# facebookresearch/jepa

Measured on AMD Instinct MI355X. Metric: V-JEPA pretrain clips/sec (fwd+bwd+EMA), higher is better.
Workload: dtype bf16; 1 GPU; V-JEPA pretrain step ViT-L/16 16x224x224, B=24/GPU, 2 multiblock masks (vitl16.yaml); global_batch=24, per_gpu_batch=24, parallelism=dp1, hw_queues=4

## Files before the change

include/vjepa_hip.h:

```cpp
#ifndef VJEPA_HIP_H
#define VJEPA_HIP_H

#include <stdint.h>

#ifdef __cplusplus
extern "C" {
#endif

typedef struct ihipStream_t* vj_stream_t;

int vj_abi_version(void);
const char* vj_last_error(void);

int vj_gather_rows(const void* src, void* dst, const int64_t* idx, int64_t B, int64_t K, int64_t row_bytes,
                   int64_t src_batch_stride_rows, vj_stream_t stream);
int vj_scatter_rows(const void* src, void* dst, const int64_t* idx, int64_t B, int64_t N, int64_t K,
                    int64_t row_bytes, vj_stream_t stream);
int vj_copy_rows(const void* src, void* dst, int64_t B, int64_t src_rows, int64_t src_off, int64_t dst_rows,
                 int64_t dst_off, int64_t n, int64_t D, vj_stream_t stream);

int vj_tubelet_pack(const float* clips, void* out_bf16, const int64_t* idx, int64_t B, int64_t C, int64_t T,
                    int64_t H, int64_t W, int64_t tubelet, int64_t patch, int64_t K, vj_stream_t stream);
int vj_add_pos(void* x_bf16, const float* pos, const int64_t* idx, int64_t B, int64_t K, int64_t D,
               vj_stream_t stream);
// ... 116 lines not shown

int vj_pred_assemble_fwd(const void* e_bf16, const float* mask_token, const float* pos, const int64_t* idx_e,
                         const int64_t* idx_p, void* out_bf16, int64_t B, int64_t Ke, int64_t Kp, int64_t D,
                         vj_stream_t stream);

int vj_target_rows(const void* x_bf16, const float* gamma, const float* beta, const int64_t* idx, float* h,
                   int64_t B, int64_t N, int64_t K, int64_t D, float eps_norm, float eps_ln, vj_stream_t stream);
int64_t vj_latent_loss_ws_bytes(void);
int vj_latent_loss(const void* z_bf16, const float* h, void* dz_bf16, int64_t numel, float p, float gscale,
                   float out_scale, int accumulate, float* loss_out, void* ws, int64_t ws_bytes,
                   vj_stream_t stream);
int vj_token_pstd(const void* z_bf16, float* pstd, float* stats ,
                  int64_t B, int64_t K, int64_t D, int accumulate, vj_stream_t stream);
int vj_reg_grad(const void* z_bf16, const float* pstd_sum, const float* stats, void* dz_bf16, int64_t B, int64_t K,
                int64_t D, int64_t n_masks, float coef, vj_stream_t stream);
int vj_reg_finish(const float* pstd_sum, int64_t n, int64_t n_masks, float* out, vj_stream_t stream);

int vj_adamw_ema(float* p, const float* g, float* exp_avg, float* exp_avg_sq, void* p_bf16, float* tgt,
                 void* tgt_bf16, int64_t n, float lr, float wd, float beta1, float beta2, float eps, int64_t step,
                 float gscale, float ema, vj_stream_t stream);
int vj_step_advance(const float* gstat, float* step_dev, vj_stream_t stream);
int vj_adamw_ema_guarded(float* p, const float* g, float* exp_avg, float* exp_avg_sq, void* p_bf16, float* tgt,
                         void* tgt_bf16, int64_t n, float lr, float wd, float beta1, float beta2, float eps, float gscale,
                         float ema, const float* gstat, int sel, float clip, float norm_scale, const float* step_dev,
                         vj_stream_t stream);
int64_t vj_grad_stats_chunks(void);
int vj_grad_stats_multi(const float* G, const float* M1, const float* M2, const int64_t* desc, int64_t n_tensors,
                        float* out, vj_stream_t stream);
int vj_ema_update(float* tgt, const float* src, void* tgt_bf16, int64_t n, float m, vj_stream_t stream);
int vj_cast_f32_to_bf16(const float* src, void* dst_bf16, int64_t n, vj_stream_t stream);
int64_t vj_sqnorm_ws_bytes(void);
int vj_sqnorm_f32(const float* g, int64_t n, float* out2, int accumulate, void* ws, int64_t ws_bytes,
                  vj_stream_t stream);

typedef struct vj_linear {
  const void* w;
  const float* b;
  const void* wT;
  int64_t ldwT;
  float* gw;
  float* gb;
  int64_t n_out, k_in;
} vj_linear_t;
typedef struct vj_norm {
  const float* g;
  const float* b;
  float* gg;
  float* gb;
} vj_norm_t;
typedef struct vj_block {
  vj_norm_t norm1;
  vj_linear_t qkv, proj;
  vj_norm_t norm2;
  vj_linear_t fc1, fc2;
} vj_block_t;
typedef void (*vj_layer_cb_t)(void* user, int layer);

int64_t vj_blocks_fwd_ws_bytes(int64_t M, int64_t D, int64_t Dh, int64_t heads, int64_t n_blocks, int save);
enum {
  VJ_GEMM_FLAGS_SEL_MASK = 0xffff,
  VJ_GEMM_FLAGS_FROM_SHIFT = 16,
  VJ_GEMM_FLAGS_FROM_MASK = 0xff
};
int vj_blocks_fwd(const vj_block_t* blocks, int64_t n_blocks, const void* x_in, void* x_out, int64_t M, int64_t D,
                  int64_t heads, const vj_seg_t* segs, int64_t n_segs, float ln_eps, int save, int gemm_flags, void* ws,
                  int64_t ws_bytes, vj_stream_t stream);
// ... 63 lines not shown
```

jepa_amd/csrc/optim.hip:

```cpp
#include "common.hpp"
#include "options.hpp"

struct AdamArgs {
  float* p;
  const float* g;
  float* m;
  float* v;
  bf16_t* p_bf16;
  float* tgt;
  bf16_t* tgt_bf16;
  int64_t n;
  float lr, wd, beta1, beta2, eps;
  float bc1, bc2_sqrt;
  float gscale;
  float ema;
  const float* gstat;
  int sel;
  float clip;
  float norm_scale;
  const float* step_dev;
};

template <bool SRC_ROUNDED>
__device__ __forceinline__ void ema4(float* tgt, bf16_t* tgt_bf16, int64_t q, float4 s, float m) {
// ... 144 lines not shown
    s += v.x * v.x + v.y * v.y + v.z * v.z + v.w * v.w;
    bad += (float)(!isfinite(v.x)) + (float)(!isfinite(v.y)) + (float)(!isfinite(v.z)) + (float)(!isfinite(v.w));
  }
  block4_stage(red, {s, bad});
  if (threadIdx.x == 0) {
    part[blockIdx.x] = block4_total(red[0]);
    part[SQ_BLOCKS + blockIdx.x] = block4_total(red[1]);
  }
}
__global__ __launch_bounds__(256) void sqnorm_finish_kernel(const float* __restrict__ part, float* __restrict__ out,
                                                            int accumulate) {
  __shared__ float red[2][4];
  float s = 0.f, bad = 0.f;
  for (int i = threadIdx.x; i < SQ_BLOCKS; i += 256) {
    s += part[i];
    bad += part[SQ_BLOCKS + i];
  }
  block4_stage(red, {s, bad});
  if (threadIdx.x == 0) {
    const float a = block4_total(red[0]), b = block4_total(red[1]);
    out[0] = accumulate ? out[0] + a : a;
    out[1] = accumulate ? out[1] + b : b;
  }
}
extern "C" int64_t vj_sqnorm_ws_bytes(void) { return 2 * SQ_BLOCKS * 4; }
extern "C" int vj_sqnorm_f32(const float* g, int64_t n, float* out2, int accumulate, void* ws, int64_t ws_bytes,
                             hipStream_t stream) {
  VJ_CHECK_ARG(n % 4 == 0, "vj_sqnorm_f32: n must be a multiple of 4");
  VJ_CHECK_ARG(ws_bytes >= vj_sqnorm_ws_bytes(), "vj_sqnorm_f32: workspace too small");
  hipLaunchKernelGGL(sqnorm_kernel, dim3(SQ_BLOCKS), dim3(256), 0, stream, g, n / 4, (float*)ws);
  VJ_LAUNCH_CHECK("vj_sqnorm_f32");
  hipLaunchKernelGGL(sqnorm_finish_kernel, dim3(1), dim3(256), 0, stream, (const float*)ws, out2, accumulate);
  VJ_LAUNCH_CHECK("vj_sqnorm_f32(finish)");
  return 0;
}

#define GS_CHUNKS 8
__global__ __launch_bounds__(256) void grad_stats_multi_kernel(const float* __restrict__ G, const float* __restrict__ M1,
                                                               const float* __restrict__ M2,
                                                               const int64_t* __restrict__ desc, float* __restrict__ out) {
  __shared__ float red[3][4];
  const int t = blockIdx.x, c = blockIdx.y;
  const int64_t off = desc[2 * t], n = desc[2 * t + 1];
  const int64_t per = cdiv64(cdiv64(n, GS_CHUNKS), 4) * 4;
  const int64_t lo = (int64_t)c * per, hi = lo + per < n ? lo + per : n;
  float s0 = 0.f, s1 = 0.f, s2 = 0.f;
  const int64_t n4 = hi > lo ? (hi - lo) >> 2 : 0;
  for (int64_t q = threadIdx.x; q < n4; q += 256) {
    const int64_t e = off + lo + 4 * q;
    const float4 g = *(const float4*)(G + e);
    s0 += g.x * g.x + g.y * g.y + g.z * g.z + g.w * g.w;
    if (M1) {
      const float4 a = *(const float4*)(M1 + e);
      const float4 b = *(const float4*)(M2 + e);
      s1 += fabsf(a.x) + fabsf(a.y) + fabsf(a.z) + fabsf(a.w);
      s2 += fabsf(b.x) + fabsf(b.y) + fabsf(b.z) + fabsf(b.w);
    }
  }
  for (int64_t e = lo + 4 * n4 + threadIdx.x; e < hi; e += 256) {
    const float g = G[off + e];
    s0 += g * g;
    if (M1) {
      s1 += fabsf(M1[off + e]);
      s2 += fabsf(M2[off + e]);
    }
  }
// ... 16 lines not shown
```

jepa_amd/engine/dp.py:

```python
import torch
import torch.distributed as dist

from .streams import independent_stream, side_stream


class GradReducer:
    def __init__(self, arena, vit, pred, world_size, overlap=True, pred_layers_per_bucket=4):
        self.arena = arena
        import os
        self.world = world_size
        self.enabled = world_size > 1 or (os.environ.get("VJ_FORCE_DP", "0") == "1" and dist.is_available()
                                          and dist.is_initialized())
        self.overlap = overlap
        self.coll_mode = os.environ.get("VJ_DP_COLL", "sync")
        if self.coll_mode not in ("sync", "async", "capi"):
            raise ValueError(f"VJ_DP_COLL={self.coll_mode!r}: expected sync, async or capi")
        self._capi = None
        self.extra_streams = []
        self.buckets = {}
        self.tail = []
        self._pending = []
        self.comm_stream = None
        self.launched = []
        self._exposed = []
        self.exposed_samples = 0
        if not self.enabled:
            return
        sl = arena.slots

        def span(prefix, names):
            offs = [sl[prefix + n] for n in names]
            return (min(s.off for s in offs), max(s.off + ((s.numel + 63) // 64) * 64 for s in offs))

        mats = ["attn.qkv.weight", "attn.proj.weight", "mlp.fc1.weight", "mlp.fc2.weight"]
        for li in range(len(vit.blocks)):
            self.buckets[("enc", li)] = [span(f"enc.blocks.{li}.", mats)]
        self.buckets[("enc", -1)] = [span("enc.", ["patch_embed.proj.weight"])]
        n_pred = len(pred.predictor_blocks)
        group = []
        for li in range(n_pred - 1, -1, -1):
            group.append(span(f"pred.predictor_blocks.{li}.", mats))
            if len(group) == pred_layers_per_bucket or li == 0:
                self.buckets[("pred", li)] = [(min(g[0] for g in group), max(g[1] for g in group))]
                group = []
        self.buckets[("pred", n_pred)] = [span("pred.", ["predictor_proj.weight"])]
        covered = sorted(r for rs in self.buckets.values() for r in rs)
        pos, total = 0, arena.total
        for lo, hi in covered:
            if lo > pos:
                self.tail.append((pos, lo))
            pos = max(pos, hi)
        if pos < total:
            self.tail.append((pos, total))
        self._diag = os.environ.get("VJ_DP_DIAG", "")
        self.coll_check = None
        if self.coll_mode == "capi" and not (arena.G.is_cuda and overlap):
            raise ValueError("VJ_DP_COLL=capi needs the gradient arena on a GPU and overlap_comm=True: the C-ABI collectives are "
                             "issued on the engine's communication stream")
        if (self.coll_mode == "capi" or self._diag == "extracomm") and arena.G.is_cuda:
            self._init_capi(arena.G.device)
            if self.coll_mode != "capi":
                self._capi_unused, self._capi = self._capi, None

    def _init_capi(self, device):
        import ctypes
        from ..hip.lib import check, load_library
        lib = load_library()
        n = lib.vj_comm_unique_id_bytes()
        idt = torch.zeros(n, dtype=torch.uint8, device=device)
        if dist.get_rank() == 0:
            buf = (ctypes.c_ubyte * n)()
            check(lib.vj_comm_unique_id(buf), "vj_comm_unique_id")
            idt.copy_(torch.tensor(list(buf), dtype=torch.uint8))
        dist.broadcast(idt, 0)
        raw = bytes(idt.cpu().tolist())
        handle = ctypes.c_void_p()
        check(lib.vj_comm_init(ctypes.byref(handle), dist.get_rank(), dist.get_world_size(), raw), "vj_comm_init")
        self._capi = (lib, handle)
        import weakref
        weakref.finalize(self, lib.vj_comm_destroy, handle)

    @property
    def route(self):
        if not (self.arena.G.is_cuda and self.overlap):
            return "blocking"
        return "capi" if self._capi is not None else self.coll_mode
# ... 79 lines not shown
            else:
                out["verdict"] = "comm-stream" if all(sid == marker for _, sid in colls) else "other-stream"
        except Exception as ex:
            out["error"] = f"{type(ex).__name__}: {ex}"[:200]
        return out

    def begin(self, producer_stream=None):
        if not self.enabled:
            return
        self.launched = []
        self._pending = []
        self._ev_next = 0
        self._producer = producer_stream
        if self.arena.G.is_cuda and self.overlap and self.comm_stream is None:
            self._pick_comm_stream()

    def _reduce(self, lo, hi, producer=None):
        g = self.arena.G[lo:hi]
        self.launched.append((lo, hi))
        if g.is_cuda and self.overlap:
            pool = self.__dict__.setdefault("_ev_pool", [])
            nxt = self.__dict__.get("_ev_next", 0)
            if nxt >= len(pool):
                pool.append(torch.cuda.Event())
            ev = pool[nxt]
            self._ev_next = nxt + 1
            ev.record(producer if producer is not None else torch.cuda.current_stream())
            self.comm_stream.wait_event(ev)
            if self._capi is not None:
                from ..hip.lib import check
                lib, handle = self._capi
                if self._diag != "skipcall":
                    check(lib.vj_comm_allreduce_bucket(handle, g.data_ptr(), g.numel(), self.comm_stream.cuda_stream), "vj_comm_allreduce_bucket")
                return
            with torch.cuda.stream(self.comm_stream):
                if self.coll_mode == "async":
                    self._pending.append(dist.all_reduce(g, op=dist.ReduceOp.SUM, async_op=True))
                else:
                    dist.all_reduce(g, op=dist.ReduceOp.SUM)
        else:
            dist.all_reduce(g, op=dist.ReduceOp.SUM)

    def layer_done(self, kind, layer):
        if not self.enabled:
            return
        for lo, hi in self.buckets.get((kind, layer), ()):
            self._reduce(lo, hi, getattr(self, "_producer", None))

    def finish(self):
        if not self.enabled:
            return
        for lo, hi in self.tail:
            self._reduce(lo, hi)
        if self.arena.G.is_cuda and self.overlap:
            cur = torch.cuda.current_stream()
            e0, e1 = torch.cuda.Event(enable_timing=True), torch.cuda.Event(enable_timing=True)
            e0.record(cur)
            for w in self._pending:
                w.wait()
            cur.wait_stream(self.comm_stream)
            e1.record(cur)
            self._exposed = (self._exposed + [(e0, e1)])[-16:]
        self._pending = []

    def exposed_ms(self):
        if not self._exposed:
            return None
        torch.cuda.synchronize()
        self.exposed_samples = len(self._exposed)
        return sum(a.elapsed_time(b) for a, b in self._exposed) / len(self._exposed)


# ... 7 lines not shown
```

jepa_amd/engine/step.py:

```python
import math
import os
import weakref

import torch

from ..hip import ops
from ..hip.lib import set_option
from . import chain, dp, optstate
from . import weights as _weights
from .layers import encoder_backward, encoder_forward, predictor_backward, predictor_forward
from .streams import device_index, independent_stream, low_priority_stream, side_stream
from .weights import FoldW, ParamArena, bump_generation, encoder_views, is_no_decay, predictor_views

_OVERLAP_FWD = os.environ.get("VJ_OVERLAP_FWD", "1") != "0"
_LN_FOLD = os.environ.get("VJ_LN_FOLD", "0") == "1"
_UPD_LOW_PRIO = os.environ.get("VJ_UPD_LOW_PRIO", "0") == "1"
_TGT_GEMM_FLAGS = int(os.environ.get("VJ_TGT_GEMM_FLAGS", "0"), 0)
_PRED_GEMM_FLAGS = int(os.environ.get("VJ_PRED_GEMM_FLAGS", "0"), 0)
_PRED_DGRAD_FLAGS = int(os.environ.get("VJ_PRED_DGRAD_FLAGS", "0"), 0)


class _TargetArena(ParamArena):

    def __init__(self, src: ParamArena, lo, hi, prefix, target_named_params, device):
        self.device = device
        self.slots = {n: s for n, s in src.slots.items() if n.startswith(prefix)}
        self.lo, self.hi = lo, hi
        self.P = torch.zeros(hi - lo, dtype=torch.float32, device=device)
        self.Pb = torch.zeros(hi - lo, dtype=torch.bfloat16, device=device)
        self.wT = {}
        self.frozen = {}
        for name, p in target_named_params:
            self.adopt(name, p)
        self.refresh_bf16()

    def make_folds(self, depth):
        self.folds = []
        for i in range(depth):
            wq, w1 = self.f32(f"enc.blocks.{i}.attn.qkv.weight"), self.f32(f"enc.blocks.{i}.mlp.fc1.weight")
            mk = lambda n: torch.empty(n, dtype=torch.float32, device=self.device)
            self.folds.append(FoldW(torch.empty_like(wq, dtype=torch.bfloat16), mk(wq.shape[0]), mk(wq.shape[0]),
                                    torch.empty_like(w1, dtype=torch.bfloat16), mk(w1.shape[0]), mk(w1.shape[0])))
        self.refresh_folds(0, depth)
        return self.folds

    def refresh_folds(self, b0, b1):
        if getattr(self, "folds", None) is None:
            return
        for i in range(b0, b1):
# ... 95 lines not shown
            if a not in self.arena.slots:
                p.data = p.data.to(device=dev, dtype=torch.float32).contiguous()
                self.tarena.frozen[a] = p.data
        self.tvit._hip_attach(self.tarena, "enc.")
        self.ew = encoder_views(self.arena, "enc.", self.vit,
                                self.arena.frozen["enc.pos_embed"].reshape(self.vit.num_patches, -1), train=True)
        self.pw = predictor_views(self.arena, "pred.", self.pred,
                                  self.arena.frozen["pred.predictor_pos_embed"].reshape(self.pred.num_patches, -1),
                                  train=True)
        self.tw = encoder_views(self.tarena, "enc.", self.tvit,
                                self.tarena.frozen["enc.pos_embed"].reshape(self.tvit.num_patches, -1), train=False)
        self._target_folds = None
        self.ln_fold_target = False
        if _LN_FOLD:
            self.set_ln_fold(True)
        def grp(named, nodecay):
            return [p for _, n, p in named if is_no_decay(n, p) == nodecay]
        self.param_groups = [
            {"params": grp(enc_named, False), "lr": 0.0, "weight_decay": 0.0, "_range": 0},
            {"params": grp(pred_named, False), "lr": 0.0, "weight_decay": 0.0, "_range": 2},
            {"params": grp(enc_named, True), "lr": 0.0, "weight_decay": 0, "WD_exclude": True, "_range": 1},
            {"params": grp(pred_named, True), "lr": 0.0, "weight_decay": 0, "WD_exclude": True, "_range": 3},
        ]
        self._slot_of = {id(sl.param): sl for sl in self.arena.slots.values()}
        self._step_dev = torch.zeros(1, dtype=torch.float32, device=dev)
        self._stat = torch.zeros(8, dtype=torch.float32, device=dev)
        self.reducer = dp.GradReducer(self.arena, self.vit, self.pred, world_size, overlap=overlap_comm)
        self.overlap_update = bool(overlap_update)
        self._upd_stream = self._make_update_stream() if self.overlap_update else None
        self.reducer.extra_streams = [self._upd_stream]
        self.reducer.prepare()
        self._gates = None
        self._plan = self._update_plan()

    @torch.no_grad()
    def forward_target(self, clips, masks_pred):
        B = clips.shape[0]
        self.tw.folds = self._target_folds if (self.ln_fold_target and self._target_folds is not None) else None
        x, _, _ = encoder_forward(self.tw, clips, None, save=False, final_norm=False, ws_tag=self._ws + "tgt",
                                  gemm_flags=_TGT_GEMM_FLAGS, gates=self._gate("enc"))
        N = self.tvit.num_patches
        return [ops.target_rows(x, self.tw.norm.g, self.tw.norm.b, mp, B, N, 1e-6, 1e-5) for mp in masks_pred]

    @torch.no_grad()
    def train_step(self, clips, masks_enc, masks_pred, lr, wd, ema, clip_now=False):
        assert len(masks_enc) == len(masks_pred), 'Currently require num encoder masks = num predictor masks'
        B = clips.shape[0]
        D = self.vit.embed_dim
        n_masks = len(masks_pred)
        mark = self._phase_mark
        mark('start')
        self._arena_stats = None
        mb = B if not self.micro_batch else min(int(self.micro_batch), B)
        chunks = [(c0, min(c0 + mb, B)) for c0 in range(0, B, mb)]
        numels = [B * mp.shape[1] * D for mp in masks_pred]
        nmin = min(numels)
        alpha = 1.0 / (nmin * n_masks)
        with_reg = self.reg_coeff != 0.0
        pstd = torch.empty((B, D), dtype=torch.float32, device=self.device)
        side = side_stream(self.device)
        hook = self.reducer.layer_done if self.reducer.enabled else None
        for ci, (c0, c1) in enumerate(chunks):
            last = ci == len(chunks) - 1
            beta = 0.0 if ci == 0 else 1.0
            cl = clips[c0:c1]
            me = [m[c0:c1] for m in masks_enc] if len(chunks) > 1 else masks_enc
            mp = [m[c0:c1] for m in masks_pred] if len(chunks) > 1 else masks_pred
            me = [m if m.is_contiguous() else m.contiguous() for m in me]
            mp = [m if m.is_contiguous() else m.contiguous() for m in mp]
            Bc = c1 - c0
            fwd_overlap = side.enabled and _OVERLAP_FWD
            if fwd_overlap:
                side.fork(cl, *mp)
                with torch.cuda.stream(side.stream):
                    h = self.forward_target(cl, mp)
            else:
                h = self.forward_target(cl, mp)
            z, segs, saved_e = encoder_forward(self.ew, cl, me, save=True, ws_tag=self._ws + "enc_save", gates=self._gate("enc"))
            zhat, tsegs, saved_p = predictor_forward(self.pw, z, segs, me, mp, save=True, ws_tag=self._ws + "pred_save",
                                                     gemm_flags=_PRED_GEMM_FLAGS, gates=self._gate("pred"))
            mark('context+predictor forward (main stream)')
            if fwd_overlap:
                side.join()
                for t in h:
                    t.record_stream(torch.cuda.current_stream())
            dzhat = torch.empty_like(zhat)
            stats = [torch.empty((Bc, D, 2), dtype=torch.float32, device=self.device) if with_reg else None
                     for _ in tsegs]
            for i, t in enumerate(tsegs):
                zi = zhat[t.row0:t.row0 + t.rows]
                ops.latent_loss(zi, h[i], self._stat[0:1], p=self.loss_exp, out_scale=1.0 / (numels[i] * n_masks),
                                accumulate=(i > 0 or ci > 0), dz=dzhat[t.row0:t.row0 + t.rows], gscale=nmin / numels[i])
                ops.token_pstd(zi, pstd[c0:c1], Bc, t.S, D, accumulate=i > 0, stats=stats[i])
            if with_reg:
                coef = self.reg_coeff / (B * D * n_masks) / alpha
                for i, t in enumerate(tsegs):
                    ops.reg_grad(zhat[t.row0:t.row0 + t.rows], pstd[c0:c1], stats[i], dzhat[t.row0:t.row0 + t.rows], Bc,
                                 t.S, D, n_masks, coef)
            mark('target forward joined + loss')
            if self._gates is not None:
                torch.cuda.current_stream().wait_event(self._gates["done"])
                self._gates = None
            if last:
                self.reducer.begin(side.stream if side.enabled else None)
            lhook = hook if last else None
            if _PRED_DGRAD_FLAGS:
                old_dg = set_option("gemm_dgrad_flags", _PRED_DGRAD_FLAGS)
            dz = predictor_backward(dzhat, saved_p, self.pw, segs, alpha, on_layer_done=lhook, beta=beta,
                                    ws_tag=self._ws + "bwd_tmp")
            if _PRED_DGRAD_FLAGS:
                set_option("gemm_dgrad_flags", old_dg)
            mark('predictor backward (main stream)')
            encoder_backward(dz, saved_e, self.ew, segs, alpha, on_layer_done=lhook, beta=beta,
                             ws_tag=self._ws + "bwd_tmp")
            mark('encoder backward (main stream)')
        ops.reg_finish(pstd, n_masks, self._stat[1:2])
        self.reducer.finish()
        clipped = bool(clip_now and self.clip_grad is not None)
        self._last_clip = float(self.clip_grad) if clipped else 0.0
        self.optimizer_step(lr, wd, ema, clip_now)
        mark('wgrad stream joined + AdamW/EMA')
        return StepOutput(self._stat.clone(), self.reg_coeff, lr, wd, ema, clipped, 1.0 / self.world_size)

    def _phase_mark(self, name):
        ev = getattr(self, 'phase_events', None)
        if ev is not None:
            e = torch.cuda.Event(enable_timing=True)
            e.record()
            ev.append((name, e))

    @property
    def opt_step(self):
        return int(self._step_dev.item())

    @opt_step.setter
    def opt_step(self, v):
        self._step_dev.fill_(float(v))

    def set_ln_fold(self, on):
        on = bool(on)
        if on:
            self.sync_update()
            if self._target_folds is None:
                self._target_folds = self.tarena.make_folds(len(self.tw.blocks))
            else:
                self.tarena.refresh_folds(0, len(self.tw.blocks))
        self.ln_fold_target = on

    def _make_update_stream(self):
        with torch.cuda.device(self.device):
            others = [torch.cuda.current_stream(self.device), side_stream(self.device).stream]
            comm = getattr(getattr(self, "reducer", None), "comm_stream", None)
            if comm is not None:
                others.append(comm)
            make = (lambda: low_priority_stream(self.device)) if _UPD_LOW_PRIO else None
# ... 21 lines not shown
                b = int(parts[2])
                return max(i for i, f in enumerate(firsts) if f <= b)
            return 0 if parts[1] == "patch_embed" else len(firsts) - 1
        plan, ok = [], True
        per_stage = [[] for _ in firsts]
        for gi in (0, 1):
            lo, hi = A.group_ranges[gi]
            slots = sorted((s for n, s in A.slots.items() if n.startswith("enc.") and lo <= s.off < hi), key=lambda s: s.off)
            stages = [stage_of(s.name) for s in slots]
            ok = ok and stages == sorted(stages) and set(stages) == set(range(len(firsts)))
            if not ok:
                break
            starts = [min(s.off for s, st in zip(slots, stages) if st == k) for k in range(len(firsts))]
            starts[0] = lo
            for k in range(len(firsts)):
                per_stage[k].append((gi, starts[k], starts[k + 1] if k + 1 < len(firsts) else hi))
        if ok:
            plan = [("enc", firsts[k], per_stage[k]) for k in range(len(firsts))]
        else:
            plan = [("enc", 0, [(gi,) + tuple(A.group_ranges[gi]) for gi in (0, 1)])]
        plan.append(("pred", 0, [(gi,) + tuple(A.group_ranges[gi]) for gi in (2, 3)]))
        return plan

    def _enc_pred_ranges(self):
        A = self.arena
        (e0, _), (_, e1) = A.group_ranges[0], A.group_ranges[1]
        (p0, _), (_, p1) = A.group_ranges[2], A.group_ranges[3]
        return (e0, e1), (p0, p1)

    def optimizer_step(self, lr, wd, ema, clip_now=False):
        A = self.arena
        inv_world = 1.0 / self.world_size
        self.sync_update()
        (e0, e1), (p0, p1) = self._enc_pred_ranges()
        ops.sqnorm(A.G[e0:e1], self._stat[4:6])
        ops.sqnorm(A.G[p0:p1], self._stat[6:8])
        gstat = self._stat[4:8]
        ops.step_advance(gstat, self._step_dev)
        clip = float(self.clip_grad) if (clip_now and self.clip_grad is not None) else 0.0
        b1, b2 = self.betas
        T = self.tarena

        def update(gi, lo, hi):
            if hi == lo:
                return
            is_enc = gi < 2
            decay = wd if gi in (0, 2) else 0.0
            tgt = T.P[lo - T.lo:hi - T.lo] if is_enc else None
            tgtb = T.Pb[lo - T.lo:hi - T.lo] if is_enc else None
            ops.adamw_ema_guarded(A.P[lo:hi], A.G[lo:hi], A.M1[lo:hi], A.M2[lo:hi], A.Pb[lo:hi], tgt, tgtb, lr, decay, b1,
                                  b2, self.eps, inv_world, ema, gstat, 0 if is_enc else 1, clip, inv_world,
                                  self._step_dev)

        if self.overlap_update and side_stream(self.device).enabled:
            main = torch.cuda.current_stream()
            ready = torch.cuda.Event()
            ready.record(main)
            if self._upd_stream is None:
                self._upd_stream = self._make_update_stream()
            upd = self._upd_stream
            upd.wait_event(ready)
            gates = {"enc": [], "pred": []}
            with torch.cuda.stream(upd):
                n_enc = sum(1 for w, _, _ in self._plan if w == "enc")
                firsts = [f for w, f, _ in self._plan if w == "enc"] + [len(self.tw.blocks)]
                for pi, (which, first_block, ranges) in enumerate(self._plan):
                    for gi, lo, hi in ranges:
                        update(gi, lo, hi)
                    if which == "enc" and self.ln_fold_target:
                        T.refresh_folds(first_block, firsts[pi + 1] if pi + 1 <= n_enc else len(self.tw.blocks))
                    ev = torch.cuda.Event()
# ... 72 lines not shown
```

jepa_amd/hip/lib.py:

```python
import ctypes
import os

import torch

_HERE = os.path.dirname(os.path.abspath(__file__))
_VARIANT = os.environ.get("VJ_LIB_VARIANT", "")
_LIB_PATH = os.path.join(os.path.dirname(_HERE), "lib", f"libvjepa_hip_{_VARIANT}.so" if _VARIANT else "libvjepa_hip.so")

P = ctypes.c_void_p
I64 = ctypes.c_int64
I32 = ctypes.c_int
F32 = ctypes.c_float
F64 = ctypes.c_double



class VjLinear(ctypes.Structure):
    _fields_ = [("w", P), ("b", P), ("wT", P), ("ldwT", I64), ("gw", P), ("gb", P), ("n_out", I64), ("k_in", I64)]


class VjNorm(ctypes.Structure):
    _fields_ = [("g", P), ("b", P), ("gg", P), ("gb", P)]


# ... 58 lines not shown
    "vj_colsum_ws_bytes": (I64, [I64]),
    "vj_colsum_bf16": (I32, [P, I64, I64, I64, I64, I64, I64, P, F32, F32, P, I64, P]),
    "vj_reduce_partials": (I32, [P, P, I64, I64, F32, F32, P]),
    "vj_reduce_segments": (I32, [P, I64, F32, F32, P]),
    "vj_attn_fwd": (I32, [P, P, P, I64, I64, I64, I64, F32, P]),
    "vj_attn_fwd_segs": (I32, [P, P, P, ctypes.POINTER(VjSeg), I64, I64, I64, F32, P]),
    "vj_attn_bwd_segs": (I32, [P, P, P, P, P, ctypes.POINTER(VjSeg), I64, I64, I64, F32, P, I64, P, P, P]),
    "vj_attn_bwd_ws_bytes": (I64, [I64, I64, I64]),
    "vj_attn_bwd_segs_ws_bytes": (I64, [ctypes.POINTER(VjSeg), I64, I64, I64]),
    "vj_attn_bwd": (I32, [P, P, P, P, P, I64, I64, I64, I64, F32, P, I64, P]),
    "vj_attn_bwd_colsum_rows": (I32, [I64, I64, I64, I64P, I64P]),
    "vj_attn_bwd_colsum": (I32, [P, P, P, P, P, I64, I64, I64, I64, F32, P, I64, P, P, P]),
    "vj_xattn_fwd": (I32, [P, I64, P, P, P, P, I64, I64, I64, I64, I64, F32, P]),
    "vj_xattn_bwd": (I32, [P, I64, P, P, P, P, P, I64, I64, I64, I64, I64, F32, P]),
    "vj_xattn_ws_bytes": (I64, [I64, I64, I64, I64, I64, I32]),
    "vj_xattn_fwd_ws": (I32, [P, I64, P, P, P, P, I64, I64, I64, I64, I64, F32, P, I64, P]),
    "vj_xattn_bwd_ws": (I32, [P, I64, P, P, P, P, P, I64, I64, I64, I64, I64, F32, P, I64, P]),
    "vj_pred_assemble_fwd": (I32, [P, P, P, P, P, P, I64, I64, I64, I64, P]),
    "vj_target_rows": (I32, [P, P, P, P, P, I64, I64, I64, I64, F32, F32, P]),
    "vj_latent_loss_ws_bytes": (I64, []),
    "vj_latent_loss": (I32, [P, P, P, I64, F32, F32, F32, I32, P, P, I64, P]),
    "vj_token_pstd": (I32, [P, P, P, I64, I64, I64, I32, P]),
    "vj_reg_grad": (I32, [P, P, P, P, I64, I64, I64, I64, F32, P]),
    "vj_reg_finish": (I32, [P, I64, I64, P, P]),
    "vj_adamw_ema": (I32, [P, P, P, P, P, P, P, I64, F32, F32, F32, F32, F32, I64, F32, F32, P]),
    "vj_step_advance": (I32, [P, P, P]),
    "vj_adamw_ema_guarded": (I32, [P, P, P, P, P, P, P, I64, F32, F32, F32, F32, F32, F32, F32, P, I32, F32, F32, P, P]),
    "vj_grad_stats_chunks": (I64, []),
    "vj_grad_stats_multi": (I32, [P, P, P, P, I64, P, P]),
    "vj_ema_update": (I32, [P, P, P, I64, F32, P]),
    "vj_cast_f32_to_bf16": (I32, [P, P, I64, P]),
    "vj_sqnorm_ws_bytes": (I64, []),
    "vj_sqnorm_f32": (I32, [P, I64, P, I32, P, I64, P]),
    "vj_blocks_fwd_ws_bytes": (I64, [I64, I64, I64, I64, I64, I32]),
    "vj_blocks_fwd": (I32, [ctypes.POINTER(VjBlock), I64, P, P, I64, I64, I64, ctypes.POINTER(VjSeg), I64, F32, I32, I32,
                            P, I64, P]),
    "vj_blocks_fwd_lnfold": (I32, [ctypes.POINTER(VjBlock), ctypes.POINTER(VjLnFold), I64, P, P, I64, I64, I64, ctypes.POINTER(VjSeg), I64,
                                   F32, I32, P, I64, P]),
    "vj_ln_rowstats": (I32, [P, P, I64, I64, F32, P]),
    "vj_ln_fold_weights": (I32, [P, P, P, P, P, P, P, I64, I64, P]),
    "vj_gemm_bf16_nt_lnfold": (I32, [P, I64, P, I64, P, I64, I64, I64, I64, P, P, P, I32, F32, I32, P]),
    "vj_blocks_bwd_ws_bytes": (I64, [I64, I64, I64, I64]),
    "vj_blocks_bwd": (I32, [ctypes.POINTER(VjBlock), I64, P, P, P, I64, I64, I64, ctypes.POINTER(VjSeg), I64, F32, F32,
                            P, I64, P, I64, I32, P, P, LAYER_CB, P]),
    "vj_prof_enable": (I32, [I32]),
    "vj_prof_collect": (I32, [F64P, F64P, I64P, ctypes.c_char_p]),
    "vj_comm_unique_id_bytes": (I64, []),
    "vj_comm_unique_id": (I32, [P]),
    "vj_comm_init": (I32, [ctypes.POINTER(P), I32, I32, P]),
    "vj_comm_allreduce_bucket": (I32, [P, P, I64, P]),
    "vj_comm_broadcast": (I32, [P, P, I64, I32, P]),
    "vj_comm_destroy": (I32, [P]),
    "vj_set_option": (I32, [ctypes.c_char_p, I32]),
    "vj_get_option": (I32, [ctypes.c_char_p, ctypes.POINTER(I32)]),
    "vj_pool_softmax_chunk_keys": (I64, []),
    "vj_pool_softmax_fwd_ws_bytes": (I64, [I64, I64, I64]),
    "vj_pool_softmax_fwd": (I32, [P, P, P, I64, I64, I64, P, I64, P]),
    "vj_pool_softmax_bwd": (I32, [P, P, P, P, I64, I64, I64, P]),
    "vj_probe_tr16": (I32, [P, I32, P]),
    "vj_probe_copy": (I32, [P, P, I64, P]),
    "vj_probe_lds_bw": (I32, [P, I32, I32, I32, P]),
    "vj_ws_guard_check": (I32, [I64P, I64P]),
    "vj_probe_spin": (I32, [I64, P]),
    "vj_probe_spin_stamped": (I32, [I64, P, P]),
}

# ... 49 lines not shown
```

jepa_amd/hip/ops.py:

```python
import ctypes
import math

import torch

from .lib import VjReduceSeg, VjSeg, check, load_library

BF16 = torch.bfloat16
F32 = torch.float32
I64 = torch.int64
I32 = torch.int32

EPI_BF16, EPI_GELU, EPI_DGELU, EPI_F32 = 0, 1, 2, 3
EPI_QKV = 4

_raw_stream = torch._C._cuda_getCurrentRawStream
_dev_index = None


def _device():
    global _dev_index
    if _dev_index is None:
        _dev_index = torch.cuda.current_device()
    return _dev_index

# ... 780 lines not shown

def grad_stats_multi(G, M1, M2, desc, n_tensors, stream=None):
    _req(G, F32, "G")
    _opt(M1, F32, "M1")
    _opt(M2, F32, "M2")
    _req(desc, I64, "desc")
    nch = _query("vj_grad_stats_chunks")
    out = torch.empty((n_tensors, nch, 3), dtype=F32, device=G.device)
    _launch("vj_grad_stats_multi", _ptr(G), _ptr(M1), _ptr(M2), _ptr(desc), n_tensors, _ptr(out), stream=stream)
    return out.sum(dim=1)


def ema_update(tgt, src, tgt_bf16, m, stream=None):
    _req(tgt, F32, "tgt")
    _req(src, F32, "src")
    _opt(tgt_bf16, BF16, "tgt_bf16")
    _launch("vj_ema_update", _ptr(tgt), _ptr(src), _ptr(tgt_bf16), tgt.numel(), m, stream=stream)


def cast_bf16(src, dst, stream=None):
    _req(src, F32, "src")
    _req(dst, BF16, "dst")
    _launch("vj_cast_f32_to_bf16", _ptr(src), _ptr(dst), src.numel(), stream=stream)
    return dst


def sqnorm(g, out2, accumulate=False, stream=None):
    _req(g, F32, "g")
    _req(out2, F32, "out2")
    nws = _query("vj_sqnorm_ws_bytes")
    ws = Scratch.get(nws, g.device, "sqnorm", stream=stream)
    _launch("vj_sqnorm_f32", _ptr(g), g.numel(), _ptr(out2), int(accumulate), _ptr(ws), nws, stream=stream)
    return out2
```

Before: 336.2 clips/s.

## Compute gradient squared norms per bucket on side stream during backward

```diff
diff --git a/include/vjepa_hip.h b/include/vjepa_hip.h
--- a/include/vjepa_hip.h
+++ b/include/vjepa_hip.h
@@ -172,6 +172,11 @@
 int64_t vj_sqnorm_ws_bytes(void);
 int vj_sqnorm_f32(const float* g, int64_t n, float* out2, int accumulate, void* ws, int64_t ws_bytes,
                   vj_stream_t stream);
+int64_t vj_sqnorm_table_bytes(int64_t n_slots);
+int64_t vj_sqnorm_bucket_adds(int64_t n);
+int vj_sqnorm_bucket_f32(const float* g, int64_t n, float* table, int64_t slot, int64_t n_slots, vj_stream_t stream);
+int vj_sqnorm_table_finish(const float* table, int64_t n_enc, int64_t n_slots, float* gstat, float* step_dev,
+                           vj_stream_t stream);
 
 typedef struct vj_linear {
   const void* w;
diff --git a/jepa_amd/csrc/optim.hip b/jepa_amd/csrc/optim.hip
--- a/jepa_amd/csrc/optim.hip
+++ b/jepa_amd/csrc/optim.hip
@@ -200,6 +200,73 @@
   VJ_LAUNCH_CHECK("vj_sqnorm_f32");
   hipLaunchKernelGGL(sqnorm_finish_kernel, dim3(1), dim3(256), 0, stream, (const float*)ws, out2, accumulate);
   VJ_LAUNCH_CHECK("vj_sqnorm_f32(finish)");
+  return 0;
+}
+
+#define SQB 256
+__global__ __launch_bounds__(256) void sqnorm_bucket_kernel(const float* __restrict__ g, int64_t n4, float* __restrict__ slot) {
+  __shared__ float red[2][4];
+  float s = 0.f, bad = 0.f;
+#pragma unroll 4
+  for (int64_t q = (int64_t)blockIdx.x * 256 + threadIdx.x; q < n4; q += (int64_t)SQB * 256) {
+    const float4 v = ((const float4*)g)[q];
+    s += v.x * v.x + v.y * v.y + v.z * v.z + v.w * v.w;
+    bad += (float)(!isfinite(v.x)) + (float)(!isfinite(v.y)) + (float)(!isfinite(v.z)) + (float)(!isfinite(v.w));
+  }
+  block4_stage(red, {s, bad});
+  if (threadIdx.x == 0) {
+    slot[blockIdx.x] = block4_total(red[0]);
+    slot[SQB + blockIdx.x] = block4_total(red[1]);
+  }
+}
+extern "C" int64_t vj_sqnorm_table_bytes(int64_t n_slots) { return n_slots * 2 * SQB * 4; }
+extern "C" int64_t vj_sqnorm_bucket_adds(int64_t n) {
+  const int64_t strides = n <= 0 ? 0 : cdiv64(n / 4, (int64_t)SQB * 256);
+  return 4 * strides + 1 + 9 + 9;
+}
+extern "C" int vj_sqnorm_bucket_f32(const float* g, int64_t n, float* table, int64_t slot, int64_t n_slots, hipStream_t stream) {
+  VJ_CHECK_ARG(g != nullptr && table != nullptr, "vj_sqnorm_bucket_f32: null pointer");
+  VJ_CHECK_ARG(n >= 0 && n % 4 == 0 && ((uintptr_t)g & 15) == 0, "vj_sqnorm_bucket_f32: the bucket must be 16-byte aligned and a multiple of 4 long");
+  VJ_CHECK_ARG(slot >= 0 && slot < n_slots, "vj_sqnorm_bucket_f32: slot %ld outside the table of %ld", (long)slot, (long)n_slots);
+  hipLaunchKernelGGL(sqnorm_bucket_kernel, dim3(SQB), dim3(256), 0, stream, g, n / 4, table + slot * 2 * SQB);
+  VJ_LAUNCH_CHECK("vj_sqnorm_bucket_f32");
+  return 0;
+}
+#define SQ_MAX_SLOTS 256
+__global__ __launch_bounds__(256) void sqnorm_table_finish_kernel(const float* __restrict__ table, int n_enc, int n_slots,
+                                                                  float* __restrict__ gstat, float* __restrict__ step_dev) {
+  __shared__ float tot[2][SQ_MAX_SLOTS];
+  const int lane = threadIdx.x & 63;
+#pragma unroll 4
+  for (int i = threadIdx.x >> 6; i < n_slots; i += 4) {
+    const float4 a = ((const float4*)(table + (int64_t)i * 2 * SQB))[lane];
+    const float4 b = ((const float4*)(table + (int64_t)i * 2 * SQB + SQB))[lane];
+    const float s = wave_sum(((a.x + a.y) + a.z) + a.w), bad = wave_sum(((b.x + b.y) + b.z) + b.w);
+    if (lane == 0) {
+      tot[0][i] = s;
+      tot[1][i] = bad;
+    }
+  }
+  __syncthreads();
+  if (threadIdx.x == 0) {
+    float out[4] = {0.f, 0.f, 0.f, 0.f};
+    for (int i = 0; i < n_slots; i++) {
+      const int m = i < n_enc ? 0 : 2;
+      out[m] += tot[0][i];
+      out[m + 1] += tot[1][i];
+    }
+    for (int k = 0; k < 4; k++) gstat[k] = out[k];
+    if (!((out[1] + out[3]) > 0.f)) *step_dev += 1.0f;
+  }
+}
+extern "C" int vj_sqnorm_table_finish(const float* table, int64_t n_enc, int64_t n_slots, float* gstat, float* step_dev,
+                                      hipStream_t stream) {
+  VJ_CHECK_ARG(table != nullptr && gstat != nullptr && step_dev != nullptr, "vj_sqnorm_table_finish: null pointer");
+  VJ_CHECK_ARG(((uintptr_t)table & 15) == 0, "vj_sqnorm_table_finish: the table must be 16-byte aligned");
+  VJ_CHECK_ARG(n_enc >= 0 && n_enc <= n_slots && n_slots <= SQ_MAX_SLOTS, "vj_sqnorm_table_finish: %ld encoder slots of %ld (at most %d)",
+               (long)n_enc, (long)n_slots, SQ_MAX_SLOTS);
+  hipLaunchKernelGGL(sqnorm_table_finish_kernel, dim3(1), dim3(256), 0, stream, table, (int)n_enc, (int)n_slots, gstat, step_dev);
+  VJ_LAUNCH_CHECK("vj_sqnorm_table_finish");
   return 0;
 }
 
diff --git a/jepa_amd/engine/dp.py b/jepa_amd/engine/dp.py
--- a/jepa_amd/engine/dp.py
+++ b/jepa_amd/engine/dp.py
@@ -2,6 +2,56 @@
 import torch.distributed as dist
 
 from .streams import independent_stream, side_stream
+
+
+def grad_buckets(slots, total, enc_depth, pred_depth, pred_layers_per_bucket=4):
+    def span(prefix, names):
+        offs = [slots[prefix + n] for n in names]
+        return (min(s.off for s in offs), max(s.off + ((s.numel + 63) // 64) * 64 for s in offs))
+
+    buckets, tail = {}, []
+    mats = ["attn.qkv.weight", "attn.proj.weight", "mlp.fc1.weight", "mlp.fc2.weight"]
+    for li in range(enc_depth):
+        buckets[("enc", li)] = [span(f"enc.blocks.{li}.", mats)]
+    buckets[("enc", -1)] = [span("enc.", ["patch_embed.proj.weight"])]
+    group = []
+    for li in range(pred_depth - 1, -1, -1):
+        group.append(span(f"pred.predictor_blocks.{li}.", mats))
+        if len(group) == pred_layers_per_bucket or li == 0:
+            buckets[("pred", li)] = [(min(g[0] for g in group), max(g[1] for g in group))]
+            group = []
+    buckets[("pred", pred_depth)] = [span("pred.", ["predictor_proj.weight"])]
+    covered = sorted(r for rs in buckets.values() for r in rs)
+    pos = 0
+    for lo, hi in covered:
+        if lo > pos:
+            tail.append((pos, lo))
+        pos = max(pos, hi)
+    if pos < total:
+        tail.append((pos, total))
+    return buckets, tail
+
+
+def norm_slots(buckets, tail, enc_range, pred_range):
+    pieces = []
+    for ranges in list(buckets.values()) + [tail]:
+        for lo, hi in ranges:
+            for mod, (r0, r1) in enumerate((enc_range, pred_range)):
+                a, b = max(lo, r0), min(hi, r1)
+                if a < b:
+                    pieces.append((mod, a, b, (lo, hi)))
+    pieces.sort(key=lambda p: p[:3])
+    pos = enc_range[0]
+    for _, a, b, src in pieces:
+        if a != pos:
+            raise ValueError(f"norm_slots: the gradient buckets do not tile the arena at {pos} (next range [{a}, {b}) of {src})")
+        pos = b
+    if enc_range[1] != pred_range[0] or pos != pred_range[1]:
+        raise ValueError(f"norm_slots: the gradient buckets end at {pos}, the parameter ranges are {enc_range} and {pred_range}")
+    by_range = {}
+    for i, (_, _, _, src) in enumerate(pieces):
+        by_range.setdefault(src, []).append(i)
+    return [(a, b) for _, a, b, _ in pieces], sum(1 for p in pieces if p[0] == 0), by_range
 
 
 class GradReducer:
@@ -22,36 +72,13 @@
         self._pending = []
         self.comm_stream = None
         self.launched = []
+        self.after_reduce = None
         self._exposed = []
         self.exposed_samples = 0
         if not self.enabled:
             return
-        sl = arena.slots
-
-        def span(prefix, names):
-            offs = [sl[prefix + n] for n in names]
-            return (min(s.off for s in offs), max(s.off + ((s.numel + 63) // 64) * 64 for s in offs))
-
-        mats = ["attn.qkv.weight", "attn.proj.weight", "mlp.fc1.weight", "mlp.fc2.weight"]
-        for li in range(len(vit.blocks)):
-            self.buckets[("enc", li)] = [span(f"enc.blocks.{li}.", mats)]
-        self.buckets[("enc", -1)] = [span("enc.", ["patch_embed.proj.weight"])]
-        n_pred = len(pred.predictor_blocks)
-        group = []
-        for li in range(n_pred - 1, -1, -1):
-            group.append(span(f"pred.predictor_blocks.{li}.", mats))
-            if len(group) == pred_layers_per_bucket or li == 0:
-                self.buckets[("pred", li)] = [(min(g[0] for g in group), max(g[1] for g in group))]
-                group = []
-        self.buckets[("pred", n_pred)] = [span("pred.", ["predictor_proj.weight"])]
-        covered = sorted(r for rs in self.buckets.values() for r in rs)
-        pos, total = 0, arena.total
-        for lo, hi in covered:
-            if lo > pos:
-                self.tail.append((pos, lo))
-            pos = max(pos, hi)
-        if pos < total:
-            self.tail.append((pos, total))
+        self.buckets, self.tail = grad_buckets(arena.slots, arena.total, len(vit.blocks), len(pred.predictor_blocks),
+                                               pred_layers_per_bucket)
         self._diag = os.environ.get("VJ_DP_DIAG", "")
         self.coll_check = None
         if self.coll_mode == "capi" and not (arena.G.is_cuda and overlap):
@@ -197,12 +224,17 @@
                 lib, handle = self._capi
                 if self._diag != "skipcall":
                     check(lib.vj_comm_allreduce_bucket(handle, g.data_ptr(), g.numel(), self.comm_stream.cuda_stream), "vj_comm_allreduce_bucket")
+                if self.after_reduce is not None:
+                    with torch.cuda.stream(self.comm_stream):
+                        self.after_reduce(lo, hi)
                 return
             with torch.cuda.stream(self.comm_stream):
                 if self.coll_mode == "async":
                     self._pending.append(dist.all_reduce(g, op=dist.ReduceOp.SUM, async_op=True))
                 else:
                     dist.all_reduce(g, op=dist.ReduceOp.SUM)
+                    if self.after_reduce is not None:
+                        self.after_reduce(lo, hi)
         else:
             dist.all_reduce(g, op=dist.ReduceOp.SUM)
 
diff --git a/jepa_amd/engine/step.py b/jepa_amd/engine/step.py
--- a/jepa_amd/engine/step.py
+++ b/jepa_amd/engine/step.py
@@ -15,6 +15,7 @@
 _OVERLAP_FWD = os.environ.get("VJ_OVERLAP_FWD", "1") != "0"
 _LN_FOLD = os.environ.get("VJ_LN_FOLD", "0") == "1"
 _UPD_LOW_PRIO = os.environ.get("VJ_UPD_LOW_PRIO", "0") == "1"
+_NORM_BUCKETS = os.environ.get("VJ_NORM_BUCKETS", "1") != "0"
 _TGT_GEMM_FLAGS = int(os.environ.get("VJ_TGT_GEMM_FLAGS", "0"), 0)
 _PRED_GEMM_FLAGS = int(os.environ.get("VJ_PRED_GEMM_FLAGS", "0"), 0)
 _PRED_DGRAD_FLAGS = int(os.environ.get("VJ_PRED_DGRAD_FLAGS", "0"), 0)
@@ -176,6 +177,16 @@
         self.reducer.prepare()
         self._gates = None
         self._plan = self._update_plan()
+        self.norm_by_bucket = _NORM_BUCKETS
+        self._norm_buckets, tail = dp.grad_buckets(self.arena.slots, self.arena.total, len(self.vit.blocks),
+                                                   len(self.pred.predictor_blocks))
+        self._norm_slots, n_enc, self._norm_by_range = dp.norm_slots(self._norm_buckets, tail, *self._enc_pred_ranges())
+        self._norm_views = [self.arena.G[lo:hi] for lo, hi in self._norm_slots]
+        self._norm_table = ops.NormTable(n_enc, len(self._norm_slots), dev)
+        self._norm_filled = set()
+        self._norm_hooks = False
+        self._norm_on_side = False
+        self.reducer.after_reduce = self._norm_fill_range
 
     @torch.no_grad()
     def forward_target(self, clips, masks_pred):
@@ -203,7 +214,7 @@
         with_reg = self.reg_coeff != 0.0
         pstd = torch.empty((B, D), dtype=torch.float32, device=self.device)
         side = side_stream(self.device)
-        hook = self.reducer.layer_done if self.reducer.enabled else None
+        hook = self._layer_done if (self.reducer.enabled or self.norm_by_bucket) else None
         for ci, (c0, c1) in enumerate(chunks):
             last = ci == len(chunks) - 1
             beta = 0.0 if ci == 0 else 1.0
@@ -247,6 +258,8 @@
                 self._gates = None
             if last:
                 self.reducer.begin(side.stream if side.enabled else None)
+                self._norm_filled.clear()
+                self._norm_hooks = self.norm_by_bucket
             lhook = hook if last else None
             if _PRED_DGRAD_FLAGS:
                 old_dg = set_option("gemm_dgrad_flags", _PRED_DGRAD_FLAGS)
@@ -260,11 +273,42 @@
             mark('encoder backward (main stream)')
         ops.reg_finish(pstd, n_masks, self._stat[1:2])
         self.reducer.finish()
+        self._norm_hooks = False
         clipped = bool(clip_now and self.clip_grad is not None)
         self._last_clip = float(self.clip_grad) if clipped else 0.0
         self.optimizer_step(lr, wd, ema, clip_now)
         mark('wgrad stream joined + AdamW/EMA')
         return StepOutput(self._stat.clone(), self.reg_coeff, lr, wd, ema, clipped, 1.0 / self.world_size)
+
+    def _layer_done(self, kind, layer):
+        if self.reducer.enabled:
+            self.reducer.layer_done(kind, layer)
+            return
+        side = side_stream(self.device)
+        if not (self._norm_hooks and side.enabled):
+            return
+        with torch.cuda.stream(side.stream):
+            for lo, hi in self._norm_buckets.get((kind, layer), ()):
+                self._norm_fill_range(lo, hi)
+        self._norm_on_side = True
+
+    def _norm_fill_range(self, lo, hi):
+        if not self._norm_hooks:
+            return
+        for i in self._norm_by_range[(lo, hi)]:
+            self._norm_table.fill(i, self._norm_views[i])
+            self._norm_filled.add(i)
+
+    def _norm_finish(self):
+        if self._norm_on_side:
+            side_stream(self.device).join()
+            self._norm_on_side = False
+        T = self._norm_table
+        for i in range(T.n_slots):
+            if i not in self._norm_filled:
+                T.fill(i, self._norm_views[i])
+        self._norm_filled.clear()
+        T.finish(self._stat[4:8], self._step_dev)
 
     def _phase_mark(self, name):
         ev = getattr(self, 'phase_events', None)
@@ -352,11 +396,14 @@
         A = self.arena
         inv_world = 1.0 / self.world_size
         self.sync_update()
-        (e0, e1), (p0, p1) = self._enc_pred_ranges()
-        ops.sqnorm(A.G[e0:e1], self._stat[4:6])
-        ops.sqnorm(A.G[p0:p1], self._stat[6:8])
         gstat = self._stat[4:8]
-        ops.step_advance(gstat, self._step_dev)
+        if self.norm_by_bucket:
+            self._norm_finish()
+        else:
+            (e0, e1), (p0, p1) = self._enc_pred_ranges()
+            ops.sqnorm(A.G[e0:e1], self._stat[4:6])
+            ops.sqnorm(A.G[p0:p1], self._stat[6:8])
+            ops.step_advance(gstat, self._step_dev)
         clip = float(self.clip_grad) if (clip_now and self.clip_grad is not None) else 0.0
         b1, b2 = self.betas
         T = self.tarena
diff --git a/jepa_amd/hip/lib.py b/jepa_amd/hip/lib.py
--- a/jepa_amd/hip/lib.py
+++ b/jepa_amd/hip/lib.py
@@ -114,6 +114,10 @@
     "vj_cast_f32_to_bf16": (I32, [P, P, I64, P]),
     "vj_sqnorm_ws_bytes": (I64, []),
     "vj_sqnorm_f32": (I32, [P, I64, P, I32, P, I64, P]),
+    "vj_sqnorm_table_bytes": (I64, [I64]),
+    "vj_sqnorm_bucket_adds": (I64, [I64]),
+    "vj_sqnorm_bucket_f32": (I32, [P, I64, P, I64, I64, P]),
+    "vj_sqnorm_table_finish": (I32, [P, I64, I64, P, P, P]),
     "vj_blocks_fwd_ws_bytes": (I64, [I64, I64, I64, I64, I64, I32]),
     "vj_blocks_fwd": (I32, [ctypes.POINTER(VjBlock), I64, P, P, I64, I64, I64, ctypes.POINTER(VjSeg), I64, F32, I32, I32,
                             P, I64, P]),
diff --git a/jepa_amd/hip/ops.py b/jepa_amd/hip/ops.py
--- a/jepa_amd/hip/ops.py
+++ b/jepa_amd/hip/ops.py
@@ -836,3 +836,27 @@
     ws = Scratch.get(nws, g.device, "sqnorm", stream=stream)
     _launch("vj_sqnorm_f32", _ptr(g), g.numel(), _ptr(out2), int(accumulate), _ptr(ws), nws, stream=stream)
     return out2
+
+
+class NormTable:
+
+    def __init__(self, n_enc, n_slots, device):
+        if not 0 <= n_enc <= n_slots:
+            raise ValueError(f"NormTable: {n_enc} encoder slots of {n_slots}")
+        self.n_enc, self.n_slots = int(n_enc), int(n_slots)
+        self.buf = torch.zeros(_query("vj_sqnorm_table_bytes", self.n_slots) // 4, dtype=F32, device=device)
+
+    @staticmethod
+    def adds(n):
+        return int(_query("vj_sqnorm_bucket_adds", int(n)))
+
+    def fill(self, slot, g, stream=None):
+        _req(g, F32, "g")
+        _launch("vj_sqnorm_bucket_f32", _ptr(g), g.numel(), _ptr(self.buf), int(slot), self.n_slots, stream=stream)
+
+    def finish(self, gstat, step_dev, stream=None):
+        _req(gstat, F32, "gstat")
+        _req(step_dev, F32, "step_dev")
+        if gstat.numel() < 4:
+            raise ValueError("gstat: needs 4 elements")
+        _launch("vj_sqnorm_table_finish", _ptr(self.buf), self.n_enc, self.n_slots, _ptr(gstat), _ptr(step_dev), stream=stream)
```

New measurement: 337.2 clips/s, median of 6. No clear change (+0.3%).
